# edward-io/torchsnapshot-1

Measured on AMD Instinct MI355X. Metric: checkpoint save GB/s + time-to-unblock, Llama-3-8B FSDP, higher is better.
Workload: dtype bf16; 1 GPU; model=Llama-3-8B, parallelism=fsdp1, checkpoint_bytes=16060522496, storage=local fs, compression=hsz1

## Files before the change

hipsnapshot/_build.py:

```python

from __future__ import annotations

import concurrent.futures
import os
import shutil
import subprocess
import sys
import tempfile

PKG_DIR = os.path.dirname(os.path.abspath(__file__))
CSRC = os.path.join(PKG_DIR, "csrc")
HSIO_SO = os.path.join(PKG_DIR, "_hsio.so")
HSGPU_SO = os.path.join(PKG_DIR, "_hsgpu.so")
HSIO_HDRS = [os.path.join(CSRC, "hsio_abi.h")]
HSGPU_HDRS = [os.path.join(CSRC, "hsgpu_abi.h"), os.path.join(CSRC, "hsgpu_hooks.h"),
              os.path.join(CSRC, "hsgpu_common.h")]
ROCM = os.environ.get("ROCM_PATH", "/opt/rocm")
SUPPORTED_ARCHS = ("gfx950",)
MAX_COMPILE_JOBS = 16


def gpu_archs(override: str = "") -> list:
    want = [a.strip() for a in (override or os.environ.get("PYTORCH_ROCM_ARCH", "")).replace(
        ",", ";").split(";") if a.strip()]
    picked = [a for a in want if a.split(":")[0] in SUPPORTED_ARCHS]
    if override and not picked:
        raise ValueError(f"--arch {override!r}: the kernels build for {SUPPORTED_ARCHS} only")
    return picked or list(SUPPORTED_ARCHS)


GPU_ARCH = gpu_archs()[0]
# ... 73 lines not shown
```

hipsnapshot/csrc/hsdma.hip:

```cpp

#include <dlfcn.h>
#include <hip/hip_runtime.h>
#include <hsa/hsa.h>
#include <hsa/hsa_ext_amd.h>

#include <algorithm>
#include <cstdint>
#include <cstdio>
#include <mutex>
#include <vector>

#include "hsgpu_common.h"

namespace {

struct HsaApi {
  decltype(&hsa_iterate_agents) iterate_agents = nullptr;
  decltype(&hsa_agent_get_info) agent_get_info = nullptr;
  decltype(&hsa_signal_create) signal_create = nullptr;
  decltype(&hsa_signal_destroy) signal_destroy = nullptr;
  decltype(&hsa_signal_store_screlease) signal_store = nullptr;
  decltype(&hsa_signal_wait_scacquire) signal_wait = nullptr;
  decltype(&hsa_amd_memory_async_copy) async_copy = nullptr;
  decltype(&hsa_amd_memory_async_copy_on_engine) async_copy_on_engine = nullptr;
  decltype(&hsa_amd_memory_copy_engine_status) engine_status = nullptr;
  bool ok = false;
};

struct DevInfo {
  hsa_agent_t gpu{0};
  hsa_agent_t cpu{0};
  uint32_t engines = 0;
  uint32_t h2d_engines = 0;
  bool ok = false;
};

std::once_flag g_once;
HsaApi g_api;
std::mutex g_mu;
std::vector<DevInfo> g_devs;
const char* g_api_err = "";

template <typename F>
bool bind(void* h, const char* name, F* out) {
  *out = reinterpret_cast<F>(dlsym(h, name));
  return *out != nullptr;
}

void load_api() {
  void* h = dlopen("libhsa-runtime64.so.1", RTLD_NOW | RTLD_NOLOAD);
// ... 92 lines not shown
    return s;
  }
  hsa_signal_t s{0};
  if (g_api.signal_create(1, 0, nullptr, &s) != HSA_STATUS_SUCCESS) {
    hs_set_error("hsa_signal_create failed");
    s.handle = 0;
  }
  return s;
}

void give_signal(hsa_signal_t s) {
  if (t_signals.size() < 16) t_signals.push_back(s);
  else g_api.signal_destroy(s);
}

int release_to_system(int dev, void* stream) {
  hipError_t e = hipSetDevice(dev);
  if (e != hipSuccess) {
    hs_set_error("hipSetDevice(%d): %s", dev, hipGetErrorString(e));
    return -2;
  }
  hipEvent_t ev;
  e = hipEventCreateWithFlags(&ev, hipEventDisableTiming | hipEventReleaseToSystem);
  if (e != hipSuccess) {
    hs_set_error("release event: %s", hipGetErrorString(e));
    return -3;
  }
  e = hipEventRecord(ev, static_cast<hipStream_t>(stream));
  if (e == hipSuccess) e = hipEventSynchronize(ev);
  (void)hipEventDestroy(ev);
  if (e != hipSuccess) {
    hs_set_error("release event: %s", hipGetErrorString(e));
    return -4;
  }
  return 0;
}

}

extern "C" {

int hsg_sdma_engines(int dev) {
  DevInfo* d = dev_info(dev);
  if (!d) return 0;
  return __builtin_popcount(d->engines);
}

int hsg_sdma_d2h(int dev, void* dst, const void* src, uint64_t n, int max_engines, void* stream) {
  DevInfo* d = dev_info(dev);
  if (!d) return -1;
// ... 16 lines not shown
    const uint64_t len = std::min(step, n - off);
    hsa_signal_t s = take_signal();
    if (s.handle == 0) {
      rc = -5;
      break;
    }
    g_api.signal_store(s, 1);
    hsa_status_t st;
    char* dp = static_cast<char*>(dst) + off;
    const char* sp = static_cast<const char*>(src) + off;
    if (k >= 1 && !engines.empty())
      st = g_api.async_copy_on_engine(dp, d->cpu, sp, d->gpu, len, 0, nullptr, s,
                                      static_cast<hsa_amd_sdma_engine_id_t>(1u << engines[i]),
                                      true);
    else
      st = g_api.async_copy(dp, d->cpu, sp, d->gpu, len, 0, nullptr, s);
    if (st != HSA_STATUS_SUCCESS) {
      give_signal(s);
      hs_set_error("hsa_amd_memory_async_copy: status 0x%x", unsigned(st));
      rc = -6;
      break;
    }
    sigs.push_back(s);
  }
  for (hsa_signal_t s : sigs) {
    const hsa_signal_value_t v =
        g_api.signal_wait(s, HSA_SIGNAL_CONDITION_LT, 1, UINT64_MAX, HSA_WAIT_STATE_BLOCKED);
    if (v < 0 && rc == 0) {
      hs_set_error("SDMA copy reported an error (%ld)", long(v));
      rc = -7;
    }
    give_signal(s);
  }
  return rc;
}

int hsg_sdma_d2h_submit(int dev, void* dst, const void* src, uint64_t n, void* stream,
                        uint64_t* handle) {
  *handle = 0;
  DevInfo* d = dev_info(dev);
  if (!d) return -1;
  if (n == 0) return 0;
  if (const int r = release_to_system(dev, stream)) return r;
  hsa_signal_t s = take_signal();
  if (s.handle == 0) return -5;
  g_api.signal_store(s, 1);
  const hsa_status_t st = g_api.async_copy(dst, d->cpu, src, d->gpu, n, 0, nullptr, s);
  if (st != HSA_STATUS_SUCCESS) {
    give_signal(s);
    hs_set_error("hsa_amd_memory_async_copy: status 0x%x", unsigned(st));
    return -6;
  }
  *handle = s.handle;
  return 0;
}

int hsg_sdma_release(int dev, void* stream) { return release_to_system(dev, stream); }

int hsg_sdma_d2h_submit_released(int dev, void* dst, const void* src, uint64_t n,
                                 uint64_t* handle) {
  *handle = 0;
  DevInfo* d = dev_info(dev);
  if (!d) return -1;
  if (n == 0) return 0;
  hsa_signal_t s = take_signal();
  if (s.handle == 0) return -5;
  g_api.signal_store(s, 1);
  const hsa_status_t st = g_api.async_copy(dst, d->cpu, src, d->gpu, n, 0, nullptr, s);
  if (st != HSA_STATUS_SUCCESS) {
    give_signal(s);
    hs_set_error("hsa_amd_memory_async_copy: status 0x%x", unsigned(st));
    return -6;
  }
  *handle = s.handle;
  return 0;
}


int hsg_sdma_h2d(int dev, void* dst, const void* src, uint64_t n) {
  DevInfo* d = dev_info(dev);
  if (!d) return -1;
  if (n == 0) return 0;
  hsa_signal_t s = take_signal();
  if (s.handle == 0) return -5;
  g_api.signal_store(s, 1);
  const hsa_status_t st = g_api.async_copy(dst, d->gpu, src, d->cpu, n, 0, nullptr, s);
  if (st != HSA_STATUS_SUCCESS) {
    give_signal(s);
    hs_set_error("hsa_amd_memory_async_copy (h2d): status 0x%x", unsigned(st));
// ... 60 lines not shown
```

hipsnapshot/csrc/hsgpu_abi.h:

```cpp

#ifndef HIPSNAPSHOT_HSGPU_ABI_H_
#define HIPSNAPSHOT_HSGPU_ABI_H_

#include <stdint.h>

enum {
  HSG_DRAIN_SYNC = 1,
  HSG_DRAIN_HASH = 2,
  HSG_DRAIN_DIRECT = 4,
  HSG_DRAIN_HASH_LOW_PRIO = 8,
  HSG_DRAIN_NICE_SHIFT = 8,
  HSG_DRAIN_PARKED_SHIFT = 16
};

enum {
  HSG_DRAIN_NUM_STATS = 9,
  HSG_DRAIN_MSG_BYTES = 256,
  HSG_RESTORE_NUM_STATS = 11,
  HSG_RESTORE_MSG_BYTES = 320
};

enum {
  HSG_CODEC_RAW = 0,
  HSG_CODEC_HSZ = 1
// ... 64 lines not shown

uint64_t hsg_hsz_meta_bytes(uint32_t n_frames);
int hsg_hsz_encode(int dev, const void* src, uint64_t logical, int w, uint32_t frame_bytes,
                   void* out, void* meta, void* total, void* stream);
int hsg_hsz_decode(int dev, const void* frames, const void* offsets, uint32_t first,
                   uint32_t count, uint64_t logical, int w, uint32_t frame_bytes, void* out,
                   void* stream, void* err);

int hsg_sdma_engines(int dev);
int hsg_sdma_d2h(int dev, void* dst, const void* src, uint64_t n, int max_engines, void* stream);
int hsg_sdma_d2h_submit(int dev, void* dst, const void* src, uint64_t n, void* stream,
                        uint64_t* handle);
int hsg_sdma_h2d(int dev, void* dst, const void* src, uint64_t n);
int hsg_sdma_h2d_submit(int dev, void* dst, const void* src, uint64_t n, uint64_t* handle);
int hsg_sdma_wait(uint64_t handle);

void hsg_rt_set_trace(int on);
void* hsg_rt_dev_alloc(int dev, uint64_t nbytes, int uncached);
void hsg_rt_dev_free(void* p);
void* hsg_rt_vmm_alloc(int dev, uint64_t nbytes, int uncached);
int hsg_rt_vmm_free(void* p);
uint64_t hsg_rt_vmm_retired_bytes();
int hsg_rt_memcpy_d2h(void* dst, const void* src, uint64_t n);

void* hsg_drain_start(int dev, int n, const uint64_t* srcs, const uint64_t* sizes,
                      const char* const* paths, uint64_t slot_bytes, int nslots, int nwriters,
                      int flags, int max_hash_grid, int* err);
int hsg_drain_wait(void* handle, uint64_t* sums, uint64_t* bytes_written, char* msg,
                   double* stats);
int hsg_drain_pending(void* handle);
void hsg_drain_boost(void* handle);

void* hsg_restore_start(int dev, int n, const char* const* paths, const uint64_t* file_lo,
                        const uint64_t* nbytes, const int* codec, const uint64_t* logical,
                        const uint64_t* direct, const uint64_t* base_off, const int64_t* desc_off,
                        const int* desc_n, const void* descs, int64_t n_descs,
                        const uint64_t* producers, int n_producers, uint32_t* err_words,
                        uint64_t slot_bytes, uint64_t first_bytes, uint64_t piece_bytes,
                        int nslots, int nreaders, uint64_t budget, int engine,
                        const int* hash_items, int hash_grid, int* err);
int hsg_restore_wait(void* handle, int* err_item, char* msg, double* stats, uint64_t* bytes_read,
                     uint64_t* sums);
int hsg_restore_prewarm(int dev, uint64_t up_bytes, uint64_t sc_bytes, uint64_t slot_bytes,
                        int nslots, uint64_t table_bytes);
uint64_t hsg_restore_trim(int dev, uint64_t keep);
uint64_t hsg_restore_trim_pools(int dev, uint64_t keep_upload, uint64_t keep_scratch);
void hsg_restore_pool_bytes(int dev, uint64_t* out);
// ... 7 lines not shown
```

hipsnapshot/csrc/hsrestore.cpp:

```cpp

#include <fcntl.h>
#include <sys/stat.h>
#include <unistd.h>

#include <algorithm>
#include <atomic>
#include <cerrno>
#include <chrono>
#include <condition_variable>
#include <cstdint>
#include <cstdio>
#include <cstdlib>
#include <cstring>
#include <deque>
#include <map>
#include <memory>
#include <mutex>
#include <string>
#include <thread>
#include <unordered_map>
#include <vector>

#include "hsgpu_hooks.h"

namespace {

constexpr uint64_t kGranule = uint64_t(2) << 20;
constexpr uint64_t kHszHeader = 64;
constexpr uint64_t kHszFrameHeader = 32;
constexpr int kRestoreSlot = 2000;

uint64_t now_ns() {
  return static_cast<uint64_t>(std::chrono::duration_cast<std::chrono::nanoseconds>(
      std::chrono::steady_clock::now().time_since_epoch()).count());
}

uint64_t align16(uint64_t n) { return (n + 15) & ~uint64_t(15); }

constexpr uint64_t kMaxRetiredVa = uint64_t(64) << 40;
struct DevPool {
// ... 196 lines not shown
  kSubmit,
  kUploadWait,
  kLaunch,
  kRetireWait,
  kFirstUpload,
  kUploadBusy,
  kWall
};
static_assert(kWall + 1 == HSG_RESTORE_NUM_STATS, "Stat and the ABI's stat count differ");

struct Job {
  int dev = 0;
  uint64_t slot_bytes = 0;
  uint64_t budget = 0;
  int engine = -1;
  std::vector<Item> items;
  std::vector<uint8_t> descs;
  uint64_t desc_size = 0;
  uint32_t* err_words = nullptr;
  void* streams[2] = {nullptr, nullptr};
  int hash_grid = 64;
  uint64_t* hash_acc = nullptr;


  std::vector<void*> slots;
  std::unique_ptr<SlotFill[]> fills;
  uint64_t piece_bytes = 0;
  int filling = -1;
  std::mutex mu;
  std::condition_variable cv;
// ... 187 lines not shown
      j->fail(rerr, i, "read");
      break;
    }
    j->bytes_read.fetch_add(pn);
    if (f.left.fetch_sub(1) != 1) continue;
    const char* sp = static_cast<const char*>(j->slots[s]);
    if (f.chunk == 0 && it.codec == HSG_CODEC_HSZ) {
      uint64_t nf = 0;
      memcpy(&nf, sp + 24, 4);
      const uint64_t hb = std::min<uint64_t>(f.n, kHszHeader + 8 * (nf + 1));
      it.head.assign(sp, sp + hb);
    }
    t0 = now_ns();
    uint64_t h = 0;
    hsg_rt_trace("upload", static_cast<char*>(it.block) + f.off, f.n, i);
    const int r = hsg_sdma_h2d_submit_on(j->dev, static_cast<char*>(it.block) + f.off, sp, f.n,
                                         j->engine, &h);
    if (!j->first_upload.exchange(true)) j->ns[kFirstUpload].store(now_ns() - j->t_start);
    j->add(kSubmit, t0);
    if (r != 0) {
      j->fail(-EIO, i, "sdma upload");
      break;
    }
    {
      std::lock_guard<std::mutex> g(j->mu);
      if (j->outstanding++ == 0) j->busy_since = now_ns();
      j->inflight.push_back(Chunk{i, f.chunk, f.off, f.n, s, h});
    }
    j->cv.notify_all();
  }
  {
    std::lock_guard<std::mutex> g(j->mu);
// ... 179 lines not shown
      if (j->retire.empty()) break;
      i = j->retire.front();
      j->retire.pop_front();
    }
    const uint64_t t0 = now_ns();
    if (hsg_rt_event_sync(j->items[i].done) != 0) j->fail(-EIO, i, "device work");
    j->add(kRetireWait, t0);
    release_item(j, j->items[i]);
  }
}

}

extern "C" {

void* hsg_restore_start(int dev, int n, const char* const* paths, const uint64_t* file_lo,
                        const uint64_t* nbytes, const int* codec, const uint64_t* logical,
                        const uint64_t* direct, const uint64_t* base_off, const int64_t* desc_off,
                        const int* desc_n, const void* descs, int64_t n_descs,
                        const uint64_t* producers, int n_producers, uint32_t* err_words,
                        uint64_t slot_bytes, uint64_t first_bytes, uint64_t piece_bytes,
                        int nslots, int nreaders, uint64_t budget, int engine,
                        const int* hash_items, int hash_grid, int* err) {
  *err = 0;
  if (hsg_rt_set_device(dev) != 0) {
    *err = -1;
    return nullptr;
  }
  Job* j = new Job();
  j->dev = dev;
  j->slot_bytes = (std::max<uint64_t>(slot_bytes, 1 << 20) + 4095) / 4096 * 4096;
  first_bytes = std::max<uint64_t>(first_bytes, 1 << 20);
  j->piece_bytes = std::min<uint64_t>(j->slot_bytes,
                                      (std::max<uint64_t>(piece_bytes, 256 << 10) + 4095) / 4096 * 4096);
  j->budget = std::max<uint64_t>(budget, kGranule);
  const uint32_t emask = hsg_sdma_h2d_engine_mask(dev);
  if (engine == -2) engine = emask ? __builtin_ctz(emask) : -1;
  j->engine = (engine >= 0 && engine < 32 && (emask & (1u << engine))) ? engine : -1;
  j->desc_size = hsg_desc_size();
  j->err_words = err_words;
  j->descs.assign(static_cast<const uint8_t*>(descs),
                  static_cast<const uint8_t*>(descs) + n_descs * int64_t(j->desc_size));
  j->items = std::vector<Item>(n);
  for (int i = 0; i < n; ++i) {
    Item& it = j->items[i];
    it.path = paths[i];
    it.file_lo = file_lo[i];
    it.nbytes = nbytes[i];
    it.codec = codec[i];
    it.logical = logical[i];
    it.direct = direct[i];
    it.base_off = base_off[i];
    it.desc_off = desc_off[i];
// ... 205 lines not shown
```

hipsnapshot/engine/native_drain.py:

```python

from __future__ import annotations

import logging
import os
import threading
import time
from typing import Dict, List, Tuple

from .. import knobs
from ..io_types import StoragePlugin, WriteReq
from ..ops import checksum, native
from ..utils.tracing import timeline

logger = logging.getLogger(__name__)


last_stats: Dict[str, float] = {}

class Booster:

    def __init__(self) -> None:
        self._lock = threading.Lock()
        self._jobs: List = []
        self.boosted = False
# ... 39 lines not shown
    return _root(storage) is not None


def split(reqs: List[WriteReq], storage: StoragePlugin) -> Tuple[List[WriteReq], List[WriteReq]]:
    if not knobs.native_drain_enabled() or not native.gpu_available() or _root(storage) is None:
        return [], list(reqs)
    nat, py = [], []
    for wr in reqs:
        (nat if eligible(wr, storage) else py).append(wr)
    return nat, py


def _run(dev: int, wrs: List[WriteReq], blobs, fsync: bool, want_sums: bool, direct: bool,
         booster: "Booster" = None):
    from ..utils.affinity import drain_thread_mask, threads_with_mask

    args = (knobs.get_drain_slot_bytes(), knobs.get_drain_slots(), knobs.get_drain_writers())
    parked = max(0, knobs.get_drain_boost_writers() - args[2])
    with threads_with_mask(drain_thread_mask(dev, knobs.drain_avoid_caller_core(),
                                             knobs.native_io_numa_local())):
        job = native.NativeDrain(dev, blobs, *args, fsync, want_sums, knobs.get_hash_grid(),
                                 knobs.get_drain_nice(), direct, knobs.drain_hash_high_priority(),
                                 parked_writers=parked)
    if booster is not None:
        booster.attach(job)
    try:
        partial, written = job.wait()
    finally:
        if booster is not None:
            booster.detach(job)
    return partial, written, job.stats, "in_process"
# ... 32 lines not shown
```

hipsnapshot/engine/native_restore.py:

```python

from __future__ import annotations

import logging
import os
import threading
import time
from collections import defaultdict
from typing import Dict, List, Optional, Tuple

import numpy as np

from .. import knobs
from ..io_types import ReadReq, StoragePlugin
from ..ops import native
from ..utils.tracing import timeline

logger = logging.getLogger(__name__)

last_stats: Dict[str, float] = {}

_RAW, _HSZ = native.CODEC_RAW, native.CODEC_HSZ


def _root(storage: StoragePlugin) -> Optional[str]:
# ... 255 lines not shown
def run(jobs: Dict[int, list], budget: Optional[int] = None, verifier=None) -> int:
    from ..ops import checksum

    _join_prewarm()
    total = 0
    slot, first, nslots = sizing(budget)
    for dev, entries in jobs.items():
        t0 = time.perf_counter()
        items = [e[1] for e in entries]
        hashed = _hash_plan(entries, verifier)
        prods = sorted({p for e in entries for p in e[2]})
        from ..utils.affinity import gpu_node_mask, threads_with_mask

        mask = gpu_node_mask(dev) if knobs.native_io_numa_local() else None
        t1 = time.perf_counter()
        with threads_with_mask(mask):
            job = native.NativeRestore(dev, items, prods, slot, knobs.get_restore_piece_bytes(),
                                       nslots, knobs.get_restore_readers(),
                                       knobs.get_restore_device_budget(),
                                       knobs.get_restore_sdma_engine(), first,
                                       hash_items=hashed, hash_grid=knobs.get_hash_grid())
        t2 = time.perf_counter()
        rc, item, msg = job.wait()
        t3 = time.perf_counter()
        bad = job.corrupt_items()
        native.restore_trim(dev, knobs.get_restore_keep_bytes())
        t4 = time.perf_counter()
        job.stats.update(py_mask=round(t1 - t0, 5), py_start=round(t2 - t1, 5),
                         py_wait=round(t3 - t2, 5), py_after=round(t4 - t3, 5))
        nbytes = sum(it[4] for it in items)
# ... 24 lines not shown
```

hipsnapshot/engine/staging.py:

```python

from __future__ import annotations

import threading
import time
from contextlib import contextmanager
from typing import Callable, Dict, Iterator, List, Optional, Sequence, Tuple

import numpy as np
import torch

from ..format.serialization import contiguous_cpu_bytes_view, tensor_from_bytes
from ..io_types import StagedBuffer, buffer_address
from ..ops import checksum, native
from ..utils.tracing import timeline

_tls = threading.local()
_slot_lock = threading.Lock()
_next_slot = [0]
NUM_COPY_SLOTS = 4
_MAX_COPY_SLOTS = 64
_DECODE_SLOT_BASE = 64
_HASH_SLOT_BASE = 128


# ... 158 lines not shown
def _hash_finish(dev: int, hslot: int, handle: int, nbytes: int) -> int:
    t_s = time.perf_counter()
    h = checksum.device_hash_result(dev, hslot, handle, nbytes)
    timeline.add("hash_wait", "d2h", t_s, time.perf_counter(), bytes=nbytes)
    return h


def _use_sdma(dev: int) -> bool:
    from .. import knobs

    if knobs.get_d2h_engine() != "sdma":
        return False
    ok = _sdma_ok.get(dev)
    if ok is None:
        ok = _sdma_ok[dev] = native.sdma_engines(dev) > 0
    return ok


def bulk_d2h(dev: int, slot: int, dst: int, src: int, nbytes: int,
             producer: Optional[int] = None) -> None:
    t_s = time.perf_counter()
    if nbytes and _use_sdma(dev):
        if producer is not None:
            native.memcpy(dev, slot, 0, 0, 0, native.D2H, producer, sync=False)
            producer = None
        try:
            native.sdma_d2h(dev, dst, src, nbytes, native.copy_stream(dev, slot))
            timeline.add("dma", "d2h", t_s, time.perf_counter(), bytes=nbytes, slot=slot)
            return
        except native.HipError as e:
            import logging
# ... 11 lines not shown
def _dma_limit(dev: int) -> threading.BoundedSemaphore:
    from .. import knobs

    n = knobs.get_dma_inflight()
    got = _dma_limits.get(dev)
    if got is None or got[0] != n:
        with _slot_lock:
            got = _dma_limits.get(dev)
            if got is None or got[0] != n:
                got = _dma_limits[dev] = (n, threading.BoundedSemaphore(n))
    return got[1]


def d2h_staged(dev: int, slot: int, staged: StagedBuffer, src: int, nbytes: int,
               keep: list, hash_handle: Optional[int] = None,
               producer: Optional[int] = None) -> None:
    from .. import knobs

    hslot = hash_slot(slot)
    if nbytes and knobs.async_dma() and _use_sdma(dev):
        if producer is not None:
            native.memcpy(dev, slot, 0, 0, 0, native.D2H, producer, sync=False)
        lim = _dma_limit(dev)
        lim.acquire()
        t_s = time.perf_counter()
        try:
            h = native.sdma_d2h_submit(dev, staged.addr, src, nbytes,
                                       native.copy_stream(dev, slot))
        except native.HipError as e:
            lim.release()
            import logging

            logging.getLogger(__name__).warning(
                f"SDMA device->host copy failed on cuda:{dev} ({e}); using hipMemcpyAsync")
            _sdma_ok[dev] = False
        else:
            done = [False]

            def ready() -> None:
                if done[0]:
                    return
                try:
                    try:
# ... 92 lines not shown
            batch.add(t.data_ptr(), t.dtype, t.stride(), pb.ptr, t.dtype,
                      _contig_strides(t.shape), list(t.shape), t.element_size())
            batch.launch(dev, native.copy_stream(dev, slot), sync=True)
    except BaseException:
        staged.release()
        raise
    timeline.add("d2h", "d2h", t_s, time.perf_counter(), bytes=nbytes, slot=slot)
    return staged


def _join_current_stream(dev: int, slot: int) -> None:
    native.memcpy(dev, slot, 0, 0, 0, native.D2H,
                  int(torch.cuda.current_stream(dev).cuda_stream), sync=False)


def _read_u64_device(dev: int, slot: int, addr: int) -> int:
    pb = native.PinnedBuffer(8)
    try:
        native.memcpy(dev, slot, pb.ptr, addr, 8, native.D2H, None, sync=True)
        return int(pb.as_tensor(8).view(torch.int64)[0])
    finally:
        pb.release()


_encode_locks: dict = {}
_encode_locks_mu = threading.Lock()


@contextmanager
def _encode_turn(dev: int, nbytes: int) -> Iterator[None]:
    from .. import knobs

    if nbytes < (256 << 20) or not knobs.serial_encode():
        yield
        return
    lock = _encode_locks.get(dev)
    if lock is None:
        with _encode_locks_mu:
            lock = _encode_locks.setdefault(dev, threading.Lock())
    with lock:
        yield


def _encode_device_to_host(dev: int, slot: int, src_u8: torch.Tensor, codec: dict
                           ) -> StagedBuffer:
    from ..ops import codec as hsz

    stream = native.copy_stream(dev, slot)
    t_s = time.perf_counter()
    try:
        with torch.cuda.device(dev):
            out, total, meta = hsz.encode_device(src_u8, int(codec["w"]), 0,
                                                 int(codec["frame_bytes"]), launch=False)
    except torch.cuda.OutOfMemoryError:
        return _encode_on_host(dev, slot, src_u8, codec)
    t_a = time.perf_counter()
    _join_current_stream(dev, slot)
    with _encode_turn(dev, src_u8.numel()):
        hsz.launch_encode(src_u8, int(codec["w"]), stream, int(codec["frame_bytes"]), out,
                          total, meta)
        t_l = time.perf_counter()
        nbytes = _read_u64_device(dev, slot, total.data_ptr())
    t_n = time.perf_counter()
    staged = _dest_staged(nbytes)
    t_p = time.perf_counter()
    timeline.add("enc_alloc", "enc", t_s, t_a)
    timeline.add("enc_launch", "enc", t_a, t_l)
    timeline.add("enc_wait", "enc", t_l, t_n)
    timeline.add("enc_pinned", "enc", t_n, t_p)
    try:
        hs = None
        if _checksums():
            hs = checksum.device_hash_start(dev, hash_slot(slot), out.data_ptr(), nbytes, slot)
        d2h_staged(dev, slot, staged, out.data_ptr(), nbytes, [out, total, meta], hs)
    except BaseException:
        staged.release()
        raise
    del out, total, meta
    timeline.add("encode_d2h", "d2h", t_s, time.perf_counter(), bytes=nbytes,
                 logical=src_u8.numel(), slot=slot)
    return staged


def _encode_on_host(dev: int, slot: int, src_u8: torch.Tensor, codec: dict) -> StagedBuffer:
    from ..ops import codec as hsz

    n = src_u8.numel()
    raw_pb = native.PinnedBuffer(max(n, 1))
    try:
        if n:
            bulk_d2h(dev, slot, raw_pb.ptr, src_u8.data_ptr(), n)
        return _encode_host_bytes(raw_pb.ptr, n, codec)
    finally:
# ... 541 lines not shown
```

hipsnapshot/knobs.py:

```python

from __future__ import annotations

import functools
import math
import os
import threading
from contextlib import contextmanager
from typing import Any, Generator, Optional

_PREFIXES = ("HIPSNAPSHOT_", "TORCHSNAPSHOT_")

MAX_CHUNK_SIZE = "MAX_CHUNK_SIZE_BYTES_OVERRIDE"
MAX_SHARD_SIZE = "MAX_SHARD_SIZE_BYTES_OVERRIDE"
SLAB_SIZE_THRESHOLD = "SLAB_SIZE_THRESHOLD_BYTES_OVERRIDE"
DISABLE_BATCHING = "DISABLE_BATCHING"
MEMORY_BUDGET = "PER_RANK_MEMORY_BUDGET_BYTES"

_DEFAULT_MAX_CHUNK_SIZE_BYTES = 512 * 1024 * 1024
_DEFAULT_MAX_SHARD_SIZE_BYTES = 512 * 1024 * 1024
_DEFAULT_SLAB_SIZE_THRESHOLD_BYTES = 128 * 1024 * 1024
MAX_PER_RANK_MEMORY_BUDGET_BYTES = 32 * 1024 * 1024 * 1024


_pins = threading.local()
# ... 114 lines not shown
    "ASYNC_HBM_STAGING", "HBM_STAGING_RESERVE_BYTES", "HBM_STAGING_MAX_BYTES", "NATIVE_DRAIN",
    "DRAIN_WRITERS", "NATIVE_RESTORE", "TRUST_OBJECTS", "REBALANCE", "STATE_DICT_BARRIERS",
    "FORCE_COLLECTIVES", "NUMA_BIND", "PINNED_POOL_MAX_BYTES", "FP8_FORMAT", "TIMELINE", "ROCTX",
)


class _Tuning:

    read_inflight = 8
    io_read_split_bytes = 8 << 20
    stage_threads = 4
    d2h_engine = "sdma"
    h2d_engine = "sdma"
    async_dma = True
    dma_inflight = 8
    serial_encode = True
    thread_staging = True
    stage_head_alone = True
    hash_grid = 64
    gpu_slab_gather = True
    slab_align = 256
    content_digests = False
    gc_after_plan = True
    plan_cache = True
    async_device_codec = "raw"
    hbm_arena_keep = True
    pinned_idle_trim_s = 300.0
    drain_slot_bytes = 64 << 20
    drain_slots = 16
    drain_nice = 10
    drain_avoid_caller_core = "core"
    drain_hash_high_priority = True
    read_head_bytes = 16 << 20
    restore_prewarm = True
    restore_plan_cache = True
    native_io_numa_local = True
    restore_slot_bytes = 128 << 20
    restore_first_bytes = 16 << 20
    restore_piece_bytes = 4 << 20
    restore_sdma_engine = -1
    restore_slots = 6
    restore_readers = 0
    restore_device_budget = 2 << 30
    restore_keep_bytes = (2 << 30) + (256 << 20)
    replica_split_min_bytes = 1 << 20
    replicated_units_per_rank = 16
    rebalance_host = False
    rebalance_min_gain = 0.1
    uvm_assume_host = None
    uvm_async_capture = True
    uvm_capture_threads = 32
    uvm_capture_overlap = False


TUNING = _Tuning()
# ... 29 lines not shown
def get_h2d_engine() -> str:
    v = str(_tuned("h2d_engine")).lower()
    if v not in ("hip", "sdma"):
        raise ValueError(f"h2d engine must be hip or sdma, not {v!r}")
    return v


def async_dma() -> bool:
    return bool(_tuned("async_dma"))


def get_dma_inflight() -> int:
    return max(1, int(_tuned("dma_inflight")))


def serial_encode() -> bool:
    return bool(_tuned("serial_encode"))


def thread_staging_enabled() -> bool:
    return bool(_tuned("thread_staging"))


def checksum_enabled() -> bool:
    return _get_bool("CHECKSUM", True)


def content_digests_enabled() -> bool:
    return bool(_tuned("content_digests"))

# ... 121 lines not shown

def native_io_numa_local() -> bool:
    return bool(_tuned("native_io_numa_local"))


def get_restore_slot_bytes() -> int:
    return max(1 << 20, int(_tuned("restore_slot_bytes")))


def get_restore_first_bytes() -> int:
    return max(1 << 20, int(_tuned("restore_first_bytes")))


def get_restore_piece_bytes() -> int:
    return max(256 << 10, int(_tuned("restore_piece_bytes")))


def get_restore_sdma_engine() -> int:
    return int(_tuned("restore_sdma_engine"))


def get_restore_slots() -> int:
    return max(2, int(_tuned("restore_slots")))


def get_restore_readers() -> int:
    v = int(_tuned("restore_readers"))
    return max(1, v) if v > 0 else max(4, min(12, get_io_threads()))


# ... 138 lines not shown
```

hipsnapshot/ops/codec.py:

```python

from __future__ import annotations

import struct
from dataclasses import dataclass
from typing import List, Tuple

import numpy as np

MAGIC = b"HSZ1"
VERSION = 2
HEADER_BYTES = 64
FRAME_HEADER_BYTES = 32
DEFAULT_FRAME_BYTES = 256 * 1024
SAMPLE = 2048
SAMPLE_RUN = 32
MAX_ESCAPES = 1024
ESC = 15
CODEC_NAME = "hsz1"
LANES = 256
LANE_TABLE_BYTES = 2 * LANES
HUFF_MAX_LEN = 11
HUFF_MAX_CODED = 65535


# ... 347 lines not shown
    return out[: h.logical_size]


def validate_offsets(h: Header, blob_len: int) -> None:
    offs = h.offsets
    if len(offs) != h.n_frames + 1 or offs[-1] > blob_len:
        raise ValueError("HSZ1 frame table out of range")
    for i in range(h.n_frames):
        lo, hi = h.frame_range(i)
        if offs[i + 1] < offs[i] + FRAME_HEADER_BYTES or offs[i + 1] - offs[i] > \
                _align16(FRAME_HEADER_BYTES + (hi - lo)):
            raise ValueError(f"HSZ1 frame {i} has an invalid size")


def encode_device(src, elem_width: int, stream_handle: int,
                  frame_bytes: int = DEFAULT_FRAME_BYTES, launch: bool = True):
    import torch

    from . import native

    logical = src.numel()
    nf = n_frames_for(logical, frame_bytes)
    out = torch.empty(max_encoded_bytes(logical, frame_bytes), dtype=torch.uint8,
                      device=src.device)
    meta = torch.empty(native.hsz_meta_bytes(nf), dtype=torch.uint8, device=src.device)
    total = torch.empty(1, dtype=torch.int64, device=src.device)
    if launch:
        launch_encode(src, elem_width, stream_handle, frame_bytes, out, total, meta)
    return out, total, meta


def launch_encode(src, elem_width: int, stream_handle: int, frame_bytes: int, out, total,
                  meta) -> None:
    import torch

    from . import native

    dev = src.device.index if src.device.index is not None else torch.cuda.current_device()
    src_addr = src.data_ptr() if src.numel() else out.data_ptr()
    native.hsz_encode_gpu(dev, src_addr, src.numel(), elem_width, frame_bytes, out.data_ptr(),
                          meta.data_ptr(), total.data_ptr(), stream_handle)


def decode_device_into(blob_dev, header: Header, out_dev, stream_handle: int,
                       first: int = 0, count: int = None, blob_base: int = 0) -> None:
    import torch

    from . import native

    count = header.n_frames - first if count is None else count
    if count <= 0:
        return
    offs = [o - blob_base for o in header.offsets[first: first + count + 1]]
    if min(offs) < 0 or offs[-1] > blob_dev.numel():
        raise ValueError("HSZ1 frames outside the device buffer")
    dev = blob_dev.device.index if blob_dev.device.index is not None else \
# ... 10 lines not shown
```

hipsnapshot/ops/native.py:

```python

from __future__ import annotations

import ctypes
import errno
import logging
import os
import threading
from typing import Dict, List, Optional, Sequence, Tuple

import numpy as np
import torch

from .. import _build

logger = logging.getLogger(__name__)

_lock = threading.Lock()
_hsio_lib: Optional[ctypes.CDLL] = None
_hsgpu_lib: Optional[ctypes.CDLL] = None
_hsgpu_error: Optional[str] = None

c_void_p = ctypes.c_void_p
c_int = ctypes.c_int
c_int64 = ctypes.c_int64
# ... 198 lines not shown
                                            c_void_p]),
    "hsg_mx8_quantize": (c_int, [c_int, c_void_p, c_int, c_int64, c_void_p, c_void_p, c_void_p]),
    "hsg_mx8_dequantize": (c_int, [c_int, c_void_p, c_void_p, c_int64, c_void_p, c_int, c_void_p]),
    "hsg_drain_start": (c_void_p, [c_int, c_int, P(c_uint64), P(c_uint64), P(c_char_p), c_uint64,
                                   c_int, c_int, c_int, c_int, P(c_int)]),
    "hsg_drain_wait": (c_int, [c_void_p, P(c_uint64), P(c_uint64), c_char_p, P(c_double)]),
    "hsg_drain_pending": (c_int, [c_void_p]),
    "hsg_drain_boost": (None, [c_void_p]),
    "hsg_restore_start": (c_void_p, [c_int, c_int, P(c_char_p), P(c_uint64), P(c_uint64), P(c_int),
                                     P(c_uint64), P(c_uint64), P(c_uint64), P(c_int64), P(c_int),
                                     c_void_p, c_int64, P(c_uint64), c_int, c_void_p, c_uint64,
                                     c_uint64, c_uint64, c_int, c_int, c_uint64, c_int, P(c_int),
                                     c_int, P(c_int)]),
    "hsg_restore_wait": (c_int, [c_void_p, P(c_int), c_char_p, P(c_double), P(c_uint64),
                                 P(c_uint64)]),
    "hsg_restore_trim": (c_uint64, [c_int, c_uint64]),
    "hsg_restore_trim_pools": (c_uint64, [c_int, c_uint64, c_uint64]),
    "hsg_restore_pool_bytes": (None, [c_int, P(c_uint64)]),
    "hsg_uncached_bytes": (c_uint64, []),
    "hsg_poison_idle_pools": (c_int, [c_int, c_int]),
    "hsg_restore_prewarm": (c_int, [c_int, c_uint64, c_uint64, c_uint64, c_int, c_uint64]),
    "hsg_sdma_h2d_submit": (c_int, [c_int, c_void_p, c_void_p, c_uint64, P(c_uint64)]),
    "hsg_is_managed": (c_int, [c_void_p]),
    "hsg_managed_location": (c_int, [c_void_p, c_uint64, P(c_int), P(c_int)]),
    "hsg_managed_place": (c_int, [c_int, c_void_p, c_uint64, c_int, c_void_p]),
    "hsg_managed_alloc": (c_void_p, [c_int, c_uint64]),
    "hsg_managed_free": (c_int, [c_void_p]),
    "hsg_gate_supported": (c_int, [c_int]),
    "hsg_gate_arm": (c_int, [c_int, c_void_p, P(c_uint32)]),
    "hsg_gate_release": (c_int, [c_int, c_uint32]),
# ... 5 lines not shown
    "hsg_sdma_engines": (c_int, [c_int]),
    "hsg_sdma_h2d": (c_int, [c_int, c_void_p, c_void_p, c_uint64]),
    "hsg_uncached_acquire": (c_void_p, [c_int, c_uint64]),
    "hsg_uncached_release": (c_int, [c_void_p]),
    "hsg_uncached_trim": (c_uint64, []),
    "hsg_rt_dev_alloc": (c_void_p, [c_int, c_uint64, c_int]),
    "hsg_rt_dev_free": (None, [c_void_p]),
    "hsg_rt_memcpy_d2h": (c_int, [c_void_p, c_void_p, c_uint64]),
    "hsg_rt_set_trace": (None, [c_int]),
    "hsg_rt_vmm_alloc": (c_void_p, [c_int, c_uint64, c_int]),
    "hsg_rt_vmm_free": (c_int, [c_void_p]),
    "hsg_rt_vmm_retired_bytes": (c_uint64, []),
    "hsg_sdma_d2h": (c_int, [c_int, c_void_p, c_void_p, c_uint64, c_int, c_void_p]),
    "hsg_sdma_d2h_submit": (c_int, [c_int, c_void_p, c_void_p, c_uint64, c_void_p, P(c_uint64)]),
    "hsg_sdma_wait": (c_int, [c_uint64]),
    "hsg_hsz_meta_bytes": (c_uint64, [c_uint32]),
    "hsg_hsz_encode": (c_int, [c_int, c_void_p, c_uint64, c_int, c_uint32, c_void_p, c_void_p,
                               c_void_p, c_void_p]),
    "hsg_hsz_decode": (c_int, [c_int, c_void_p, c_void_p, c_uint32, c_uint32, c_uint64, c_int,
                               c_uint32, c_void_p, c_void_p, c_void_p]),
}


def _load_hsgpu() -> Optional[ctypes.CDLL]:
    global _hsgpu_lib, _hsgpu_error
    if _hsgpu_lib is not None or _hsgpu_error is not None:
        return _hsgpu_lib
    with _lock:
        if _hsgpu_lib is not None or _hsgpu_error is not None:
            return _hsgpu_lib
# ... 183 lines not shown

def uncached_trim() -> int:
    return int(require_gpu_lib().hsg_uncached_trim())


def sdma_d2h_submit(dev: int, dst: int, src: int, nbytes: int, stream=None) -> int:
    h = c_uint64(0)
    _check(require_gpu_lib().hsg_sdma_d2h_submit(dev, dst, src, nbytes,
                                                 _stream_handle(stream) or None, ctypes.byref(h)),
           "hsg_sdma_d2h_submit")
    return h.value


def sdma_wait(handle: int) -> None:
    _check(require_gpu_lib().hsg_sdma_wait(handle), "hsg_sdma_wait")


def copy_stream(dev: int, slot: int) -> int:
    h = require_gpu_lib().hsg_copy_stream(dev, slot)
    if not h:
        raise HipError("hsg_copy_stream failed")
    return h


def stream_join(dev: int, slot: int, consumer) -> None:
    _check(require_gpu_lib().hsg_stream_join(dev, slot, _stream_handle(consumer)),
           "hsg_stream_join")


def stream_sync(dev: int, slot: int) -> None:
# ... 579 lines not shown
```

Before: 79.46 GB/s.

## Write encoded size to pinned host word and add SDMA lane striping

The compressed encode path now has the kernel write its output size straight into a pooled pinned host word. After a release-to-system event sync, the host reads that word, which replaces the separate 8-byte device-to-host memcpy round trip. The following D2H submit then skips a second release sync, and release events are pooled instead of being created and destroyed each time. The change also adds round-robin striping of D2H and H2D copies across several SDMA engines (D2H defaults to 1 lane, so that part is off; H2D restore defaults to 2), with a fallback to the default engine on error. The risks are memory-visibility correctness when reading the host word and contention between engines.

```diff
diff --git a/hipsnapshot/_build.py b/hipsnapshot/_build.py
--- a/hipsnapshot/_build.py
+++ b/hipsnapshot/_build.py
@@ -14,7 +14,8 @@
 HSGPU_SO = os.path.join(PKG_DIR, "_hsgpu.so")
 HSIO_HDRS = [os.path.join(CSRC, "hsio_abi.h")]
 HSGPU_HDRS = [os.path.join(CSRC, "hsgpu_abi.h"), os.path.join(CSRC, "hsgpu_hooks.h"),
-              os.path.join(CSRC, "hsgpu_common.h")]
+              os.path.join(CSRC, "hsgpu_common.h"),
+              os.path.join(CSRC, "sdma_lanes.h")]
 ROCM = os.environ.get("ROCM_PATH", "/opt/rocm")
 SUPPORTED_ARCHS = ("gfx950",)
 MAX_COMPILE_JOBS = 16
diff --git a/hipsnapshot/csrc/hsdma.hip b/hipsnapshot/csrc/hsdma.hip
--- a/hipsnapshot/csrc/hsdma.hip
+++ b/hipsnapshot/csrc/hsdma.hip
@@ -11,6 +11,7 @@
 #include <vector>
 
 #include "hsgpu_common.h"
+#include "sdma_lanes.h"
 
 namespace {
 
@@ -34,6 +35,13 @@
   uint32_t h2d_engines = 0;
   bool ok = false;
 };
+
+constexpr int kLaneDevs = 64;
+struct DevLanes {
+  std::atomic<int> want{1};
+  hs::LaneSet set;
+};
+DevLanes g_d2h_lanes[kLaneDevs];
 
 std::once_flag g_once;
 HsaApi g_api;
@@ -156,26 +164,62 @@
   else g_api.signal_destroy(s);
 }
 
+thread_local std::vector<std::vector<hipEvent_t>> t_release_events;
+
 int release_to_system(int dev, void* stream) {
   hipError_t e = hipSetDevice(dev);
   if (e != hipSuccess) {
     hs_set_error("hipSetDevice(%d): %s", dev, hipGetErrorString(e));
     return -2;
   }
+  if (int(t_release_events.size()) <= dev) t_release_events.resize(dev + 1);
+  std::vector<hipEvent_t>& pool = t_release_events[dev];
   hipEvent_t ev;
-  e = hipEventCreateWithFlags(&ev, hipEventDisableTiming | hipEventReleaseToSystem);
-  if (e != hipSuccess) {
-    hs_set_error("release event: %s", hipGetErrorString(e));
-    return -3;
+  if (!pool.empty()) {
+    ev = pool.back();
+    pool.pop_back();
+  } else {
+    e = hipEventCreateWithFlags(&ev, hipEventDisableTiming | hipEventReleaseToSystem);
+    if (e != hipSuccess) {
+      hs_set_error("release event: %s", hipGetErrorString(e));
+      return -3;
+    }
   }
   e = hipEventRecord(ev, static_cast<hipStream_t>(stream));
   if (e == hipSuccess) e = hipEventSynchronize(ev);
-  (void)hipEventDestroy(ev);
   if (e != hipSuccess) {
+    (void)hipEventDestroy(ev);
     hs_set_error("release event: %s", hipGetErrorString(e));
     return -4;
   }
-  return 0;
+  if (pool.size() < 4) pool.push_back(ev);
+  else (void)hipEventDestroy(ev);
+  return 0;
+}
+
+int apply_lanes(int dev, const DevInfo* d) {
+  DevLanes& L = g_d2h_lanes[dev];
+  const int k = L.set.set(d->engines, L.want.load());
+  return k < 2 ? 1 : k;
+}
+
+hsa_status_t submit_d2h(int dev, const DevInfo* d, void* dst, const void* src, uint64_t n,
+                        hsa_signal_t s) {
+  if (dev < kLaneDevs) {
+    DevLanes& L = g_d2h_lanes[dev];
+    const int engine = L.set.pick();
+    if (engine >= 0) {
+      const hsa_status_t st = g_api.async_copy_on_engine(
+          dst, d->cpu, src, d->gpu, n, 0, nullptr, s,
+          static_cast<hsa_amd_sdma_engine_id_t>(1u << engine), true);
+      if (st == HSA_STATUS_SUCCESS) return st;
+      hs_set_error("hsa_amd_memory_async_copy_on_engine(%d): status 0x%x; lanes off", engine,
+                   unsigned(st));
+      L.want.store(1);
+      L.set.set(0, 0);
+    }
+  }
+  return g_api.async_copy(dst, d->cpu, src, d->gpu, n, 0, nullptr, s);
 }
 
 }
@@ -222,7 +266,7 @@
                                       static_cast<hsa_amd_sdma_engine_id_t>(1u << engines[i]),
                                       true);
     else
-      st = g_api.async_copy(dp, d->cpu, sp, d->gpu, len, 0, nullptr, s);
+      st = submit_d2h(dev, d, dp, sp, len, s);
     if (st != HSA_STATUS_SUCCESS) {
       give_signal(s);
       hs_set_error("hsa_amd_memory_async_copy: status 0x%x", unsigned(st));
@@ -253,7 +297,7 @@
   hsa_signal_t s = take_signal();
   if (s.handle == 0) return -5;
   g_api.signal_store(s, 1);
-  const hsa_status_t st = g_api.async_copy(dst, d->cpu, src, d->gpu, n, 0, nullptr, s);
+  const hsa_status_t st = submit_d2h(dev, d, dst, src, n, s);
   if (st != HSA_STATUS_SUCCESS) {
     give_signal(s);
     hs_set_error("hsa_amd_memory_async_copy: status 0x%x", unsigned(st));
@@ -274,13 +318,87 @@
   hsa_signal_t s = take_signal();
   if (s.handle == 0) return -5;
   g_api.signal_store(s, 1);
-  const hsa_status_t st = g_api.async_copy(dst, d->cpu, src, d->gpu, n, 0, nullptr, s);
+  const hsa_status_t st = submit_d2h(dev, d, dst, src, n, s);
   if (st != HSA_STATUS_SUCCESS) {
     give_signal(s);
     hs_set_error("hsa_amd_memory_async_copy: status 0x%x", unsigned(st));
     return -6;
   }
   *handle = s.handle;
+  return 0;
+}
+
+int hsg_sdma_d2h_submit_after_release(int dev, void* dst, const void* src, uint64_t n,
+                                      uint64_t* handle) {
+  return hsg_sdma_d2h_submit_released(dev, dst, src, n, handle);
+}
+
+int hsg_sdma_d2h_lanes(int dev, int n) {
+  DevInfo* d = dev_info(dev);
+  if (!d) return -1;
+  if (dev >= kLaneDevs) return 1;
+  g_d2h_lanes[dev].want.store(n);
+  return apply_lanes(dev, d);
+}
+
+
+namespace {
+
+constexpr size_t kWordBytes = 64;
+constexpr size_t kWordPage = 4096;
+
+std::mutex g_words_mu;
+std::vector<void*> g_words;
+
+struct WordCache {
+  std::vector<void*> free;
+  ~WordCache() {
+    std::lock_guard<std::mutex> g(g_words_mu);
+    g_words.insert(g_words.end(), free.begin(), free.end());
+  }
+};
+thread_local WordCache t_words;
+
+}
+
+void* hsg_size_word_acquire() {
+  void* w = nullptr;
+  if (!t_words.free.empty()) {
+    w = t_words.free.back();
+    t_words.free.pop_back();
+  } else {
+    std::lock_guard<std::mutex> g(g_words_mu);
+    if (g_words.empty()) {
+      void* page = nullptr;
+      const hipError_t e = hipHostMalloc(&page, kWordPage, hipHostMallocDefault);
+      if (e != hipSuccess) {
+        hs_set_error("hipHostMalloc(size words): %s", hipGetErrorString(e));
+        return nullptr;
+      }
+      for (size_t off = 0; off < kWordPage; off += kWordBytes)
+        g_words.push_back(static_cast<char*>(page) + off);
+    }
+    w = g_words.back();
+    g_words.pop_back();
+  }
+  *static_cast<volatile uint64_t*>(w) = 0;
+  return w;
+}
+
+void hsg_size_word_release(void* word) {
+  if (word == nullptr) return;
+  if (t_words.free.size() < 4) {
+    t_words.free.push_back(word);
+    return;
+  }
+  std::lock_guard<std::mutex> g(g_words_mu);
+  g_words.push_back(word);
+}
+
+int hsg_size_word_wait(int dev, void* stream, const void* word, uint64_t* value) {
+  *value = 0;
+  if (const int r = release_to_system(dev, stream)) return r;
+  *value = __atomic_load_n(static_cast<const uint64_t*>(word), __ATOMIC_ACQUIRE);
   return 0;
 }
 
diff --git a/hipsnapshot/csrc/hsgpu_abi.h b/hipsnapshot/csrc/hsgpu_abi.h
--- a/hipsnapshot/csrc/hsgpu_abi.h
+++ b/hipsnapshot/csrc/hsgpu_abi.h
@@ -102,6 +102,12 @@
 int hsg_sdma_h2d(int dev, void* dst, const void* src, uint64_t n);
 int hsg_sdma_h2d_submit(int dev, void* dst, const void* src, uint64_t n, uint64_t* handle);
 int hsg_sdma_wait(uint64_t handle);
+int hsg_sdma_d2h_lanes(int dev, int n);
+int hsg_sdma_d2h_submit_after_release(int dev, void* dst, const void* src, uint64_t n,
+                                      uint64_t* handle);
+void* hsg_size_word_acquire();
+void hsg_size_word_release(void* word);
+int hsg_size_word_wait(int dev, void* stream, const void* word, uint64_t* value);
 
 void hsg_rt_set_trace(int on);
 void* hsg_rt_dev_alloc(int dev, uint64_t nbytes, int uncached);
@@ -119,6 +125,7 @@
 int hsg_drain_pending(void* handle);
 void hsg_drain_boost(void* handle);
 
+int hsg_restore_h2d_lanes(int n);
 void* hsg_restore_start(int dev, int n, const char* const* paths, const uint64_t* file_lo,
                         const uint64_t* nbytes, const int* codec, const uint64_t* logical,
                         const uint64_t* direct, const uint64_t* base_off, const int64_t* desc_off,
diff --git a/hipsnapshot/csrc/hsrestore.cpp b/hipsnapshot/csrc/hsrestore.cpp
--- a/hipsnapshot/csrc/hsrestore.cpp
+++ b/hipsnapshot/csrc/hsrestore.cpp
@@ -22,8 +22,11 @@
 #include <vector>
 
 #include "hsgpu_hooks.h"
+#include "sdma_lanes.h"
 
 namespace {
+
+std::atomic<int> g_h2d_lanes{2};
 
 constexpr uint64_t kGranule = uint64_t(2) << 20;
 constexpr uint64_t kHszHeader = 64;
@@ -250,6 +253,7 @@
   uint64_t slot_bytes = 0;
   uint64_t budget = 0;
   int engine = -1;
+  hs::LaneSet lanes;
   std::vector<Item> items;
   std::vector<uint8_t> descs;
   uint64_t desc_size = 0;
@@ -467,8 +471,14 @@
     t0 = now_ns();
     uint64_t h = 0;
     hsg_rt_trace("upload", static_cast<char*>(it.block) + f.off, f.n, i);
-    const int r = hsg_sdma_h2d_submit_on(j->dev, static_cast<char*>(it.block) + f.off, sp, f.n,
-                                         j->engine, &h);
+    const int lane = j->engine >= 0 ? -1 : j->lanes.pick();
+    int r = hsg_sdma_h2d_submit_on(j->dev, static_cast<char*>(it.block) + f.off, sp, f.n,
+                                   lane >= 0 ? lane : j->engine, &h);
+    if (r != 0 && lane >= 0) {
+      g_h2d_lanes.store(1);
+      j->lanes.set(0, 0);
+      r = hsg_sdma_h2d_submit_on(j->dev, static_cast<char*>(it.block) + f.off, sp, f.n, -1, &h);
+    }
     if (!j->first_upload.exchange(true)) j->ns[kFirstUpload].store(now_ns() - j->t_start);
     j->add(kSubmit, t0);
     if (r != 0) {
@@ -678,6 +688,12 @@
 
 extern "C" {
 
+int hsg_restore_h2d_lanes(int n) {
+  n = std::max(1, std::min(n, hs::kMaxLanes));
+  g_h2d_lanes.store(n);
+  return n;
+}
+
 void* hsg_restore_start(int dev, int n, const char* const* paths, const uint64_t* file_lo,
                         const uint64_t* nbytes, const int* codec, const uint64_t* logical,
                         const uint64_t* direct, const uint64_t* base_off, const int64_t* desc_off,
@@ -700,7 +716,9 @@
   j->budget = std::max<uint64_t>(budget, kGranule);
   const uint32_t emask = hsg_sdma_h2d_engine_mask(dev);
   if (engine == -2) engine = emask ? __builtin_ctz(emask) : -1;
+  const bool own_choice = engine == -1;
   j->engine = (engine >= 0 && engine < 32 && (emask & (1u << engine))) ? engine : -1;
+  if (own_choice) j->lanes.set(emask, g_h2d_lanes.load());
   j->desc_size = hsg_desc_size();
   j->err_words = err_words;
   j->descs.assign(static_cast<const uint8_t*>(descs),
diff --git a/hipsnapshot/csrc/sdma_lanes.h b/hipsnapshot/csrc/sdma_lanes.h
--- /dev/null
+++ b/hipsnapshot/csrc/sdma_lanes.h
@@ -0,0 +1,45 @@
+
+#ifndef HIPSNAPSHOT_SDMA_LANES_H_
+#define HIPSNAPSHOT_SDMA_LANES_H_
+
+#include <atomic>
+#include <cstdint>
+
+namespace hs {
+
+constexpr int kMaxLanes = 3;
+
+inline int lowest_engines(uint32_t mask, int want, int* lanes) {
+  int n = 0;
+  if (want > kMaxLanes) want = kMaxLanes;
+  for (int b = 0; b < 32 && n < want; ++b)
+    if (mask & (1u << b)) lanes[n++] = b;
+  return n;
+}
+
+struct LaneSet {
+  std::atomic<int> n{0};
+  std::atomic<int> engine[kMaxLanes]{};
+  std::atomic<uint32_t> next{0};
+
+  int set(uint32_t mask, int want) {
+    int e[kMaxLanes] = {0, 0, 0};
+    int k = lowest_engines(mask, want, e);
+    if (k < 2) k = 0;
+    n.store(0, std::memory_order_release);
+    for (int i = 0; i < k; ++i) engine[i].store(e[i], std::memory_order_relaxed);
+    n.store(k, std::memory_order_release);
+    return k;
+  }
+
+  int pick() {
+    const int k = n.load(std::memory_order_acquire);
+    if (k < 2) return -1;
+    const uint32_t i = next.fetch_add(1, std::memory_order_relaxed);
+    return engine[i % uint32_t(k)].load(std::memory_order_relaxed);
+  }
+};
+
+}
+
+#endif
diff --git a/hipsnapshot/engine/native_drain.py b/hipsnapshot/engine/native_drain.py
--- a/hipsnapshot/engine/native_drain.py
+++ b/hipsnapshot/engine/native_drain.py
@@ -77,7 +77,9 @@
 def _run(dev: int, wrs: List[WriteReq], blobs, fsync: bool, want_sums: bool, direct: bool,
          booster: "Booster" = None):
     from ..utils.affinity import drain_thread_mask, threads_with_mask
+    from .staging import apply_d2h_lanes
 
+    apply_d2h_lanes(dev)
     args = (knobs.get_drain_slot_bytes(), knobs.get_drain_slots(), knobs.get_drain_writers())
     parked = max(0, knobs.get_drain_boost_writers() - args[2])
     with threads_with_mask(drain_thread_mask(dev, knobs.drain_avoid_caller_core(),
diff --git a/hipsnapshot/engine/native_restore.py b/hipsnapshot/engine/native_restore.py
--- a/hipsnapshot/engine/native_restore.py
+++ b/hipsnapshot/engine/native_restore.py
@@ -293,6 +293,7 @@
 
         mask = gpu_node_mask(dev) if knobs.native_io_numa_local() else None
         t1 = time.perf_counter()
+        native.restore_h2d_lanes(knobs.get_h2d_lanes())
         with threads_with_mask(mask):
             job = native.NativeRestore(dev, items, prods, slot, knobs.get_restore_piece_bytes(),
                                        nslots, knobs.get_restore_readers(),
diff --git a/hipsnapshot/engine/staging.py b/hipsnapshot/engine/staging.py
--- a/hipsnapshot/engine/staging.py
+++ b/hipsnapshot/engine/staging.py
@@ -196,7 +196,22 @@
     ok = _sdma_ok.get(dev)
     if ok is None:
         ok = _sdma_ok[dev] = native.sdma_engines(dev) > 0
+    if ok:
+        apply_d2h_lanes(dev)
     return ok
+
+
+_d2h_lanes: dict = {}
+
+
+def apply_d2h_lanes(dev: int) -> None:
+    from .. import knobs
+
+    n = knobs.get_d2h_lanes()
+    if _d2h_lanes.get(dev) != n:
+        if native.sdma_engines(dev) > 0:
+            native.sdma_d2h_lanes(dev, n)
+        _d2h_lanes[dev] = n
 
 
 def bulk_d2h(dev: int, slot: int, dst: int, src: int, nbytes: int,
@@ -238,7 +253,7 @@
 
 def d2h_staged(dev: int, slot: int, staged: StagedBuffer, src: int, nbytes: int,
                keep: list, hash_handle: Optional[int] = None,
-               producer: Optional[int] = None) -> None:
+               producer: Optional[int] = None, released: bool = False) -> None:
     from .. import knobs
 
     hslot = hash_slot(slot)
@@ -249,8 +264,11 @@
         lim.acquire()
         t_s = time.perf_counter()
         try:
-            h = native.sdma_d2h_submit(dev, staged.addr, src, nbytes,
-                                       native.copy_stream(dev, slot))
+            if released and producer is None:
+                h = native.sdma_d2h_submit_after_release(dev, staged.addr, src, nbytes)
+            else:
+                h = native.sdma_d2h_submit(dev, staged.addr, src, nbytes,
+                                           native.copy_stream(dev, slot))
         except native.HipError as e:
             lim.release()
             import logging
@@ -373,15 +391,6 @@
                   int(torch.cuda.current_stream(dev).cuda_stream), sync=False)
 
 
-def _read_u64_device(dev: int, slot: int, addr: int) -> int:
-    pb = native.PinnedBuffer(8)
-    try:
-        native.memcpy(dev, slot, pb.ptr, addr, 8, native.D2H, None, sync=True)
-        return int(pb.as_tensor(8).view(torch.int64)[0])
-    finally:
-        pb.release()
-
-
 _encode_locks: dict = {}
 _encode_locks_mu = threading.Lock()
 
@@ -409,17 +418,20 @@
     t_s = time.perf_counter()
     try:
         with torch.cuda.device(dev):
-            out, total, meta = hsz.encode_device(src_u8, int(codec["w"]), 0,
-                                                 int(codec["frame_bytes"]), launch=False)
+            out, _, meta = hsz.encode_device(src_u8, int(codec["w"]), 0,
+                                             int(codec["frame_bytes"]), launch=False,
+                                             device_total=False)
     except torch.cuda.OutOfMemoryError:
         return _encode_on_host(dev, slot, src_u8, codec)
+    word = native.SizeWord()
     t_a = time.perf_counter()
     _join_current_stream(dev, slot)
     with _encode_turn(dev, src_u8.numel()):
         hsz.launch_encode(src_u8, int(codec["w"]), stream, int(codec["frame_bytes"]), out,
-                          total, meta)
+                          word.ptr, meta)
         t_l = time.perf_counter()
-        nbytes = _read_u64_device(dev, slot, total.data_ptr())
+        nbytes = word.wait(dev, stream)
+    word.release()
     t_n = time.perf_counter()
     staged = _dest_staged(nbytes)
     t_p = time.perf_counter()
@@ -431,11 +443,11 @@
         hs = None
         if _checksums():
             hs = checksum.device_hash_start(dev, hash_slot(slot), out.data_ptr(), nbytes, slot)
-        d2h_staged(dev, slot, staged, out.data_ptr(), nbytes, [out, total, meta], hs)
+        d2h_staged(dev, slot, staged, out.data_ptr(), nbytes, [out, meta], hs, released=True)
     except BaseException:
         staged.release()
         raise
-    del out, total, meta
+    del out, meta
     timeline.add("encode_d2h", "d2h", t_s, time.perf_counter(), bytes=nbytes,
                  logical=src_u8.numel(), slot=slot)
     return staged
diff --git a/hipsnapshot/knobs.py b/hipsnapshot/knobs.py
--- a/hipsnapshot/knobs.py
+++ b/hipsnapshot/knobs.py
@@ -152,6 +152,7 @@
     h2d_engine = "sdma"
     async_dma = True
     dma_inflight = 8
+    d2h_lanes = 1
     serial_encode = True
     thread_staging = True
     stage_head_alone = True
@@ -177,6 +178,7 @@
     restore_first_bytes = 16 << 20
     restore_piece_bytes = 4 << 20
     restore_sdma_engine = -1
+    h2d_lanes = 2
     restore_slots = 6
     restore_readers = 0
     restore_device_budget = 2 << 30
@@ -236,6 +238,10 @@
     return max(1, int(_tuned("dma_inflight")))
 
 
+def get_d2h_lanes() -> int:
+    return max(1, int(_tuned("d2h_lanes")))
+
+
 def serial_encode() -> bool:
     return bool(_tuned("serial_encode"))
 
@@ -387,6 +393,10 @@
 
 def get_restore_piece_bytes() -> int:
     return max(256 << 10, int(_tuned("restore_piece_bytes")))
+
+
+def get_h2d_lanes() -> int:
+    return max(1, int(_tuned("h2d_lanes")))
 
 
 def get_restore_sdma_engine() -> int:
diff --git a/hipsnapshot/ops/codec.py b/hipsnapshot/ops/codec.py
--- a/hipsnapshot/ops/codec.py
+++ b/hipsnapshot/ops/codec.py
@@ -385,7 +385,8 @@
 
 
 def encode_device(src, elem_width: int, stream_handle: int,
-                  frame_bytes: int = DEFAULT_FRAME_BYTES, launch: bool = True):
+                  frame_bytes: int = DEFAULT_FRAME_BYTES, launch: bool = True,
+                  device_total: bool = True):
     import torch
 
     from . import native
@@ -395,7 +396,7 @@
     out = torch.empty(max_encoded_bytes(logical, frame_bytes), dtype=torch.uint8,
                       device=src.device)
     meta = torch.empty(native.hsz_meta_bytes(nf), dtype=torch.uint8, device=src.device)
-    total = torch.empty(1, dtype=torch.int64, device=src.device)
+    total = torch.empty(1, dtype=torch.int64, device=src.device) if device_total else None
     if launch:
         launch_encode(src, elem_width, stream_handle, frame_bytes, out, total, meta)
     return out, total, meta
@@ -410,7 +411,8 @@
     dev = src.device.index if src.device.index is not None else torch.cuda.current_device()
     src_addr = src.data_ptr() if src.numel() else out.data_ptr()
     native.hsz_encode_gpu(dev, src_addr, src.numel(), elem_width, frame_bytes, out.data_ptr(),
-                          meta.data_ptr(), total.data_ptr(), stream_handle)
+                          meta.data_ptr(),
+                          total if isinstance(total, int) else total.data_ptr(), stream_handle)
 
 
 def decode_device_into(blob_dev, header: Header, out_dev, stream_handle: int,
diff --git a/hipsnapshot/ops/native.py b/hipsnapshot/ops/native.py
--- a/hipsnapshot/ops/native.py
+++ b/hipsnapshot/ops/native.py
@@ -236,6 +236,7 @@
                                      c_int, P(c_int)]),
     "hsg_restore_wait": (c_int, [c_void_p, P(c_int), c_char_p, P(c_double), P(c_uint64),
                                  P(c_uint64)]),
+    "hsg_restore_h2d_lanes": (c_int, [c_int]),
     "hsg_restore_trim": (c_uint64, [c_int, c_uint64]),
     "hsg_restore_trim_pools": (c_uint64, [c_int, c_uint64, c_uint64]),
     "hsg_restore_pool_bytes": (None, [c_int, P(c_uint64)]),
@@ -271,6 +272,12 @@
     "hsg_sdma_d2h": (c_int, [c_int, c_void_p, c_void_p, c_uint64, c_int, c_void_p]),
     "hsg_sdma_d2h_submit": (c_int, [c_int, c_void_p, c_void_p, c_uint64, c_void_p, P(c_uint64)]),
     "hsg_sdma_wait": (c_int, [c_uint64]),
+    "hsg_sdma_d2h_lanes": (c_int, [c_int, c_int]),
+    "hsg_sdma_d2h_submit_after_release": (c_int, [c_int, c_void_p, c_void_p, c_uint64,
+                                                  P(c_uint64)]),
+    "hsg_size_word_acquire": (c_void_p, []),
+    "hsg_size_word_release": (None, [c_void_p]),
+    "hsg_size_word_wait": (c_int, [c_int, c_void_p, c_void_p, P(c_uint64)]),
     "hsg_hsz_meta_bytes": (c_uint64, [c_uint32]),
     "hsg_hsz_encode": (c_int, [c_int, c_void_p, c_uint64, c_int, c_uint32, c_void_p, c_void_p,
                                c_void_p, c_void_p]),
@@ -484,6 +491,48 @@
 
 def sdma_wait(handle: int) -> None:
     _check(require_gpu_lib().hsg_sdma_wait(handle), "hsg_sdma_wait")
+
+
+def sdma_d2h_submit_after_release(dev: int, dst: int, src: int, nbytes: int) -> int:
+    h = c_uint64(0)
+    _check(require_gpu_lib().hsg_sdma_d2h_submit_after_release(dev, dst, src, nbytes,
+                                                               ctypes.byref(h)),
+           "hsg_sdma_d2h_submit_after_release")
+    return h.value
+
+
+def restore_h2d_lanes(n: int) -> int:
+    return int(require_gpu_lib().hsg_restore_h2d_lanes(int(n)))
+
+
+def sdma_d2h_lanes(dev: int, n: int) -> int:
+    r = int(require_gpu_lib().hsg_sdma_d2h_lanes(dev, int(n)))
+    if r < 0:
+        _check(r, "hsg_sdma_d2h_lanes")
+    return r
+
+
+class SizeWord:
+
+    __slots__ = ("ptr",)
+
+    def __init__(self) -> None:
+        lib = require_gpu_lib()
+        self.ptr = lib.hsg_size_word_acquire()
+        if not self.ptr:
+            raise HipError(f"hsg_size_word_acquire failed: {lib.hsg_last_error().decode()}")
+
+    def wait(self, dev: int, stream) -> int:
+        v = c_uint64(0)
+        _check(require_gpu_lib().hsg_size_word_wait(dev, _stream_handle(stream) or None,
+                                                    self.ptr, ctypes.byref(v)),
+               "hsg_size_word_wait")
+        return v.value
+
+    def release(self) -> None:
+        ptr, self.ptr = self.ptr, None
+        if ptr:
+            require_gpu_lib().hsg_size_word_release(ptr)
 
 
 def copy_stream(dev: int, slot: int) -> int:
```

Result: no change. 79.99 GB/s (median of 6 runs) (+0.7%).
